# FangjinhuaWang/PatchmatchNet

Hardware: AMD Instinct MI355X
Metric: depth-maps/sec at 1600x1200 N=5 src views (higher is better)
Workload: dtype f32

## Files before the change

### patchmatchnet_amd/csrc/conv_f16s.hip

```cpp
#include "conv_common.hpp"

struct F16sArgs {
    int N, H, W, Ho, Wo, relu;
    int cout, ca;
    float* out_b;
};

template <int CIN, int COUT, int KS, int S, int CC, int CCP, int MT, int WPS, int DIL = 1, int OUTMODE = 0, bool SWAP = (OUTMODE == 0)>
__global__ __launch_bounds__(256, WPS) void conv_f16s_kernel(const float* __restrict__ in, const f16x8* __restrict__ wB,
                                                             const float* __restrict__ shift, float* __restrict__ out,
                                                             const F16sArgs a) {
    constexpr int NT = COUT / 16, NCB = CC / 8, CHUNKS = CIN / CC, NQ = KS * KS * NCB, KSTEPS = (NQ + 3) / 4;
    constexpr int TH = 4 * MT, TW = 16, PH = (TH - 1) * S + (KS - 1) * DIL + 1, PW = (TW - 1) * S + (KS - 1) * DIL + 1;
    constexpr int PAD = DIL * (KS / 2);
    constexpr int PLANE = PH * PW * CCP;
    constexpr int NTHR = 256;
    static_assert(!SWAP || OUTMODE == 0, "swapped operand roles (see the epilogue) serve the channels-last output");
    static_assert(CCP % 8 == 0 && CC % 8 == 0 && CIN % CC == 0, "16-byte aligned channel blocks");
    extern __shared__ float4 f16s_lds4[];
    _Float16* Phi = reinterpret_cast<_Float16*>(f16s_lds4);
    _Float16* Plo = Phi + PLANE;
    const int tid = threadIdx.x, wave = __builtin_amdgcn_readfirstlane(tid >> 6), lane = tid & 63, li = lane & 15, kb = lane >> 4;
    const int tiles_x = (a.Wo + TW - 1) / TW, tiles_y = (a.Ho + TH - 1) / TH;
    const int bt = pmn_xcd_tile(blockIdx.x, a.N * tiles_x * tiles_y);
    const int n = bt / (tiles_x * tiles_y), tr = bt - n * tiles_x * tiles_y;
    const int oy0 = (tr / tiles_x) * TH, ox0 = (tr % tiles_x) * TW;
    const int iy0 = oy0 * S - PAD, ix0 = ox0 * S - PAD;

    f32x4_t accM[MT][NT], accL[MT][NT];
#pragma unroll
    for (int t = 0; t < MT; ++t)
#pragma unroll
        for (int nt = 0; nt < NT; ++nt) {
            accM[t][nt] = f32x4_t{0.f, 0.f, 0.f, 0.f};
            accL[t][nt] = f32x4_t{0.f, 0.f, 0.f, 0.f};
        }

    const f16x8* bl = wB + lane;
    f16x8 bq[2][NT][2];
#pragma unroll
    for (int nt = 0; nt < NT; ++nt) {
        bq[0][nt][0] = bl[(size_t)((0 * NT + nt) * 2 + 0) * 64];
        bq[0][nt][1] = bl[(size_t)((0 * NT + nt) * 2 + 1) * 64];
    }

    const int q4x4 = 4 * (tid % (CC / 4)), pix_first = tid / (CC / 4);
    const int py_first = pix_first / PW, px_first = pix_first - py_first * PW, lds_first = pix_first * CCP + q4x4;

#pragma unroll 1
    for (int ch = 0; ch < CHUNKS; ++ch) {
        if (ch) __syncthreads();
        {
            constexpr int QP = CC / 4, TOT = PH * PW * QP, NL = (TOT + NTHR - 1) / NTHR, SB = 6;
            constexpr int DPIX = NTHR / QP, DY = DPIX / PW, DX = DPIX - DY * PW;
            static_assert(NTHR % QP == 0, "a step of NTHR units is a whole number of pixels");
            const float* src = in + (size_t)n * a.H * a.W * CIN + ch * CC;
            int py = py_first, px = px_first;
#pragma unroll
            for (int k0 = 0; k0 < NL; k0 += SB) {
                float4 v[SB];
#pragma unroll
                for (int k = 0; k < SB; ++k) {
                    const int gy = iy0 + py, gx = ix0 + px;
                    v[k] = make_float4(0.f, 0.f, 0.f, 0.f);
                    if (k0 + k < NL && tid < TOT - (k0 + k) * NTHR && (unsigned)gy < (unsigned)a.H && (unsigned)gx < (unsigned)a.W)
                        v[k] = *reinterpret_cast<const float4*>(src + ((unsigned)(gy * a.W + gx) * CIN + q4x4));
                    px += DX;
                    py += DY;
                    if (px >= PW) {
                        px -= PW;
                        ++py;
                    }
                }
#pragma unroll
                for (int k = 0; k < SB; ++k) {
                    if (k0 + k < NL && tid < TOT - (k0 + k) * NTHR) {
                        f16x4 hi, lo;
                        f16s_split4(v[k], hi, lo);
                        *reinterpret_cast<f16x4*>(Phi + lds_first + (k0 + k) * DPIX * CCP) = hi;
                        *reinterpret_cast<f16x4*>(Plo + lds_first + (k0 + k) * DPIX * CCP) = lo;
                    }
                }
            }
        }
        __syncthreads();

#pragma unroll
        for (int ks = 0; ks < KSTEPS; ++ks) {
            const int cur = ks & 1, nxt = cur ^ 1;
            {
                const int step = ch * KSTEPS + ks + 1;
                const int lim = CHUNKS * KSTEPS - 1;
                const int sidx = step < lim ? step : lim;
#pragma unroll
                for (int nt = 0; nt < NT; ++nt) {
                    bq[nxt][nt][0] = bl[(size_t)((sidx * NT + nt) * 2 + 0) * 64];
                    bq[nxt][nt][1] = bl[(size_t)((sidx * NT + nt) * 2 + 1) * 64];
                }
            }
            int q = 4 * ks + kb;
            if (4 * ks + 3 >= NQ) q = q < NQ - 1 ? q : NQ - 1;
            const int tap = q / NCB, cb = q - tap * NCB;
            const int dy = tap / KS, dx = tap - dy * KS;
            const _Float16* pa = Phi + ((wave * MT * S + dy * DIL) * PW + li * S + dx * DIL) * CCP + cb * 8;
            f16x8 ah[MT], al[MT];
#pragma unroll
            for (int t = 0; t < MT; ++t) {
                ah[t] = *reinterpret_cast<const f16x8*>(pa + t * S * PW * CCP);
                al[t] = *reinterpret_cast<const f16x8*>(pa + t * S * PW * CCP + PLANE);
            }
#pragma unroll
            for (int t = 0; t < MT; ++t)
#pragma unroll
                for (int nt = 0; nt < NT; ++nt)
                    accM[t][nt] = SWAP ? __builtin_amdgcn_mfma_f32_16x16x32_f16(bq[cur][nt][0], ah[t], accM[t][nt], 0, 0, 0)
                                       : __builtin_amdgcn_mfma_f32_16x16x32_f16(ah[t], bq[cur][nt][0], accM[t][nt], 0, 0, 0);
#pragma unroll
            for (int t = 0; t < MT; ++t)
#pragma unroll
                for (int nt = 0; nt < NT; ++nt)
                    accL[t][nt] = SWAP ? __builtin_amdgcn_mfma_f32_16x16x32_f16(bq[cur][nt][1], ah[t], accL[t][nt], 0, 0, 0)
                                       : __builtin_amdgcn_mfma_f32_16x16x32_f16(ah[t], bq[cur][nt][1], accL[t][nt], 0, 0, 0);
#pragma unroll
            for (int t = 0; t < MT; ++t)
#pragma unroll
                for (int nt = 0; nt < NT; ++nt)
                    accL[t][nt] = SWAP ? __builtin_amdgcn_mfma_f32_16x16x32_f16(bq[cur][nt][0], al[t], accL[t][nt], 0, 0, 0)
                                       : __builtin_amdgcn_mfma_f32_16x16x32_f16(al[t], bq[cur][nt][0], accL[t][nt], 0, 0, 0);
            __builtin_amdgcn_sched_barrier(0);
        }
        if (KSTEPS & 1) {
#pragma unroll
            for (int nt = 0; nt < NT; ++nt) {
                bq[0][nt][0] = bq[1][nt][0];
                bq[0][nt][1] = bq[1][nt][1];
            }
        }
    }

    if constexpr (SWAP) {
        const int ox = ox0 + li, oyw = oy0 + wave * MT;
        if (ox < a.Wo) {
            float* po = out + (((size_t)n * a.Ho + oyw) * a.Wo + ox) * COUT + 4 * kb;
            const size_t rs = (size_t)a.Wo * COUT;
            f32x4_t sh[NT];
#pragma unroll
            for (int nt = 0; nt < NT; ++nt) sh[nt] = *reinterpret_cast<const f32x4_t*>(shift + 16 * nt + 4 * kb);
#pragma unroll
            for (int t = 0; t < MT; ++t) {
                if (oyw + t < a.Ho) {
#pragma unroll
                    for (int nt = 0; nt < NT; ++nt) {
                        f32x4_t v = f16s_epilogue(accM[t][nt], accL[t][nt], sh[nt]);
                        if (a.relu) v = f16s_relu(v);
                        *reinterpret_cast<f32x4_t*>(po + t * rs + 16 * nt) = v;
                    }
                }
            }
        }
        return;
    }
#pragma unroll
    for (int nt = 0; nt < NT; ++nt) {
        const int c = nt * 16 + li;
        const float sh = shift[c];
#pragma unroll
        for (int t = 0; t < MT; ++t) {
            const int oy = oy0 + wave * MT + t;
            float v[4];
#pragma unroll
            for (int r = 0; r < 4; ++r) {
                v[r] = f16s_epilogue(accM[t][nt][r], accL[t][nt][r], sh);
                if (a.relu) v[r] = fmaxf(v[r], 0.0f);
            }
            if constexpr (OUTMODE == 0) {
#pragma unroll
                for (int r = 0; r < 4; ++r) {
                    const int ox = ox0 + 4 * kb + r;
                    if (oy < a.Ho && ox < a.Wo) out[(((size_t)n * a.Ho + oy) * a.Wo + ox) * COUT + c] = v[r];
                }
            } else {
                if (c < a.cout && oy < a.Ho) {
                    const bool first = c < a.ca;
                    float* dst = first ? out : a.out_b;
                    const int cx = first ? c : c - a.ca, nc = first ? a.ca : a.cout - a.ca;
                    if constexpr (OUTMODE == 1) {
                        float* row = dst + (((size_t)n * nc + cx) * a.Ho + oy) * a.Wo;
                        const int ox = ox0 + 4 * kb;
                        if ((a.Wo & 3) == 0 && ox + 3 < a.Wo) {
                            *reinterpret_cast<float4*>(row + ox) = make_float4(v[0], v[1], v[2], v[3]);
                        } else {
#pragma unroll
                            for (int r = 0; r < 4; ++r)
                                if (ox + r < a.Wo) row[ox + r] = v[r];
                        }
                    } else {
#pragma unroll
                        for (int r = 0; r < 4; ++r) {
                            const int ox = ox0 + 4 * kb + r;
                            if (ox < a.Wo) dst[(((size_t)n * a.Ho + oy) * a.Wo + ox) * nc + cx] = v[r];
                        }
                    }
                }
            }
        }
    }
}

template <int CIN, int COUT, int KS, int S, int CC, int CCP, int MT, int WPS, int DIL = 1, int OUTMODE = 0, bool SWAP = (OUTMODE == 0)>
static int launch_f16s(const float* in, const void* w, const float* shift, float* out, F16sArgs a, hipStream_t st) {
    constexpr int TH = 4 * MT, PH = (TH - 1) * S + (KS - 1) * DIL + 1, PW = 15 * S + (KS - 1) * DIL + 1;
    const size_t lds = (size_t)2 * PH * PW * CCP * sizeof(_Float16);
    auto kern = conv_f16s_kernel<CIN, COUT, KS, S, CC, CCP, MT, WPS, DIL, OUTMODE, SWAP>;
    if ((size_t)a.H * a.W * CIN >= ((size_t)1 << 30)) return PMN_ERR_SHAPE;
    if (lds > 48 * 1024 && pmn_raise_dynamic_lds(reinterpret_cast<const void*>(kern), lds) != PMN_OK) return PMN_ERR_LAUNCH;
    const int blocks = a.N * ((a.Wo + 15) / 16) * ((a.Ho + TH - 1) / TH);
    PMN_LAUNCH(kern, dim3(blocks), dim3(256), lds, st, in, reinterpret_cast<const f16x8*>(w), shift, out, a);
    PMN_CHECK_LAUNCH();
    return PMN_OK;
}

extern "C" int pmn_conv2d_f16s(const float* in, const void* weights, const float* shift, float* out, int N, int H, int W, int cin,
                               int cout, int k, int stride, int relu, void* stream) {
    if (!in || !weights || !shift || !out || N < 1 || H < 1 || W < 1) return PMN_ERR_ARG;
    F16sArgs a;
    a.N = N; a.H = H; a.W = W; a.relu = relu;
    a.cout = cout; a.ca = cout; a.out_b = nullptr;
    a.Ho = (H - 1) / (stride > 0 ? stride : 1) + 1;
    a.Wo = (W - 1) / (stride > 0 ? stride : 1) + 1;
    hipStream_t st = (hipStream_t)stream;
    if (k == 3 && stride == 1 && cin == 16 && cout == 16) return launch_f16s<16, 16, 3, 1, 16, 16, 4, 4>(in, weights, shift, out, a, st);
    if (k == 3 && stride == 1 && cin == 32 && cout == 32) return launch_f16s<32, 32, 3, 1, 16, 16, 2, 4, 1, 0, false>(in, weights, shift, out, a, st);
    if (k == 3 && stride == 1 && cin == 64 && cout == 64) return launch_f16s<64, 64, 3, 1, 16, 16, 2, 3>(in, weights, shift, out, a, st);
    if (k == 5 && stride == 2 && cin == 8 && cout == 16) return launch_f16s<8, 16, 5, 2, 8, 8, 2, 4>(in, weights, shift, out, a, st);
    if (k == 5 && stride == 2 && cin == 16 && cout == 32) return launch_f16s<16, 32, 5, 2, 8, 8, 2, 4, 1, 0, false>(in, weights, shift, out, a, st);
    if (k == 5 && stride == 2 && cin == 32 && cout == 64) return launch_f16s<32, 64, 5, 2, 16, 24, 2, 2>(in, weights, shift, out, a, st);
    return PMN_ERR_SHAPE;
}


template <int WPS>
__global__ __launch_bounds__(256, WPS) void conv_f16s_pair16_kernel(const float* __restrict__ in, const f16x8* __restrict__ wA,
                                                                   const float* __restrict__ shiftA, const f16x8* __restrict__ wBq,
                                                                   const float* __restrict__ shiftB, float* __restrict__ out,
                                                                   const F16sArgs a) {
    constexpr int C = 16, CCP = 16, NCB = 2, NQ = 18, KSTEPS = 5, TO = 14, RA = 16, PI = 18;
    constexpr int PLANE = PI * PI * CCP;
    extern __shared__ float4 f16s_pair_lds4[];
    _Float16* Phi = reinterpret_cast<_Float16*>(f16s_pair_lds4);
    _Float16* Plo = Phi + PLANE;
    const int tid = threadIdx.x, wave = __builtin_amdgcn_readfirstlane(tid >> 6), lane = tid & 63, li = lane & 15, kb = lane >> 4;
    const int tiles_x = (a.W + TO - 1) / TO, tiles_y = (a.H + TO - 1) / TO;
    const int bt = pmn_xcd_tile(blockIdx.x, a.N * tiles_x * tiles_y);
    const int n = bt / (tiles_x * tiles_y), tr = bt - n * tiles_x * tiles_y;
    const int oy0 = (tr / tiles_x) * TO, ox0 = (tr % tiles_x) * TO;

    {
        constexpr int QP = C / 4, TOT = PI * PI * QP, NL = (TOT + 255) / 256;
        const float* src = in + (size_t)n * a.H * a.W * C;
        float4 v[NL];
#pragma unroll
        for (int k = 0; k < NL; ++k) {
            const int idx = tid + k * 256, pix = idx / QP, q = idx - pix * QP;
            const int py = pix / PI, px = pix - py * PI, gy = oy0 - 2 + py, gx = ox0 - 2 + px;
            v[k] = make_float4(0.f, 0.f, 0.f, 0.f);
            if (idx < TOT && (unsigned)gy < (unsigned)a.H && (unsigned)gx < (unsigned)a.W)
                v[k] = *reinterpret_cast<const float4*>(src + ((unsigned)(gy * a.W + gx) * C + 4 * q));
        }
#pragma unroll
        for (int k = 0; k < NL; ++k) {
            const int idx = tid + k * 256, pix = idx / QP, q = idx - pix * QP;
            if (idx < TOT) {
                f16x4 hi, lo;
                f16s_split4(v[k], hi, lo);
                *reinterpret_cast<f16x4*>(Phi + pix * CCP + 4 * q) = hi;
                *reinterpret_cast<f16x4*>(Plo + pix * CCP + 4 * q) = lo;
            }
        }
    }
    __syncthreads();

    f32x4_t accM[4], accL[4];
    auto layer = [&](const f16x8* __restrict__ wq, const int pitch) {
        const f16x8* bl = wq + lane;
        f16x8 bq[2][2];
        bq[0][0] = bl[0];
        bq[0][1] = bl[64];
#pragma unroll
        for (int t = 0; t < 4; ++t) {
            accM[t] = f32x4_t{0.f, 0.f, 0.f, 0.f};
            accL[t] = f32x4_t{0.f, 0.f, 0.f, 0.f};
        }
#pragma unroll
        for (int ks = 0; ks < KSTEPS; ++ks) {
            const int cur = ks & 1, nxt = cur ^ 1;
            const int sidx = ks + 1 < KSTEPS ? ks + 1 : KSTEPS - 1;
            bq[nxt][0] = bl[(size_t)(sidx * 2 + 0) * 64];
            bq[nxt][1] = bl[(size_t)(sidx * 2 + 1) * 64];
            int q = 4 * ks + kb;
            if (4 * ks + 3 >= NQ) q = q < NQ - 1 ? q : NQ - 1;
            const int tap = q / NCB, cb = q - tap * NCB;
            const int dy = tap / 3, dx = tap - dy * 3;
            const _Float16* pa = Phi + ((wave * 4 + dy) * pitch + li + dx) * CCP + cb * 8;
            f16x8 ah[4], al[4];
#pragma unroll
            for (int t = 0; t < 4; ++t) {
                ah[t] = *reinterpret_cast<const f16x8*>(pa + t * pitch * CCP);
                al[t] = *reinterpret_cast<const f16x8*>(pa + t * pitch * CCP + PLANE);
            }
#pragma unroll
            for (int t = 0; t < 4; ++t) accM[t] = __builtin_amdgcn_mfma_f32_16x16x32_f16(bq[cur][0], ah[t], accM[t], 0, 0, 0);
#pragma unroll
            for (int t = 0; t < 4; ++t) accL[t] = __builtin_amdgcn_mfma_f32_16x16x32_f16(bq[cur][1], ah[t], accL[t], 0, 0, 0);
#pragma unroll
            for (int t = 0; t < 4; ++t) accL[t] = __builtin_amdgcn_mfma_f32_16x16x32_f16(bq[cur][0], al[t], accL[t], 0, 0, 0);
            __builtin_amdgcn_sched_barrier(0);
        }
    };

    layer(wA, PI);
    f16x4 rh[4], rl[4];
    {
        const f32x4_t sh = *reinterpret_cast<const f32x4_t*>(shiftA + 4 * kb);
        const int gx = ox0 - 1 + li;
#pragma unroll
        for (int t = 0; t < 4; ++t) {
            const int gy = oy0 - 1 + wave * 4 + t;
            f32x4_t v = f16s_epilogue(accM[t], accL[t], sh);
            if (a.relu) v = f16s_relu(v);
            if (!((unsigned)gy < (unsigned)a.H && (unsigned)gx < (unsigned)a.W)) v = f32x4_t{0.f, 0.f, 0.f, 0.f};
            f16s_split4(v, rh[t], rl[t]);
        }
    }
    __syncthreads();
#pragma unroll
    for (int t = 0; t < 4; ++t) {
        const int pix = (wave * 4 + t) * RA + li;
        *reinterpret_cast<f16x4*>(Phi + pix * CCP + 4 * kb) = rh[t];
        *reinterpret_cast<f16x4*>(Plo + pix * CCP + 4 * kb) = rl[t];
    }
    __syncthreads();

    layer(wBq, RA);
    {
        const int ox = ox0 + li;
        if (li < TO && ox < a.W) {
            const f32x4_t sh = *reinterpret_cast<const f32x4_t*>(shiftB + 4 * kb);
#pragma unroll
            for (int t = 0; t < 4; ++t) {
                const int r = wave * 4 + t, oy = oy0 + r;
                if (r < TO && oy < a.H) {
                    f32x4_t v = f16s_epilogue(accM[t], accL[t], sh);
                    if (a.relu) v = f16s_relu(v);
                    *reinterpret_cast<f32x4_t*>(out + (((size_t)n * a.H + oy) * a.W + ox) * C + 4 * kb) = v;
                }
            }
        }
    }
}

extern "C" int pmn_conv2d_f16s_pair(const float* in, const void* weights_a, const float* shift_a, const void* weights_b,
                                    const float* shift_b, float* out, int N, int H, int W, int channels, int relu, void* stream) {
    if (!in || !weights_a || !shift_a || !weights_b || !shift_b || !out || N < 1 || H < 1 || W < 1) return PMN_ERR_ARG;
    if (channels != 16) return PMN_ERR_SHAPE;
    if ((size_t)H * W * 16 >= ((size_t)1 << 30)) return PMN_ERR_SHAPE;
    F16sArgs a;
    a.N = N; a.H = H; a.W = W; a.Ho = H; a.Wo = W; a.relu = relu;
    a.cout = 16; a.ca = 16; a.out_b = nullptr;
    const size_t lds = (size_t)2 * 18 * 18 * 16 * sizeof(_Float16);
    const int blocks = N * ((W + 13) / 14) * ((H + 13) / 14);
    PMN_LAUNCH(conv_f16s_pair16_kernel<4>, dim3(blocks), dim3(256), lds, (hipStream_t)stream, in, reinterpret_cast<const f16x8*>(weights_a),
               shift_a, reinterpret_cast<const f16x8*>(weights_b), shift_b, out, a);
    PMN_CHECK_LAUNCH();
    return PMN_OK;
}


template <int CIN, int DIL, int MT, int WPS>
static int dispatch_heads(const float* in, const void* w, const float* shift, float* out_a, int coutp, F16sArgs a, hipStream_t st) {
    if (coutp == 32) return launch_f16s<CIN, 32, 3, 1, 16, 16, MT, WPS, DIL, 1>(in, w, shift, out_a, a, st);
    if (coutp == 48) return launch_f16s<CIN, 48, 3, 1, 16, 16, MT, WPS, DIL, 1>(in, w, shift, out_a, a, st);
    if (coutp == 64) return launch_f16s<CIN, 64, 3, 1, 16, 16, MT, (WPS > 3 ? 3 : WPS), DIL, 1>(in, w, shift, out_a, a, st);
    return PMN_ERR_SHAPE;
}

extern "C" int pmn_offset_heads_f16s(const float* in, const void* weights, const float* shift, float* out_a, float* out_b, int N, int H,
                                     int W, int cin, int cout, int ca, int dil, void* stream) {
    if (!in || !weights || !shift || !out_a || N < 1 || H < 1 || W < 1 || cout < 1 || ca < 1 || ca > cout) return PMN_ERR_ARG;
    if (ca < cout && !out_b) return PMN_ERR_ARG;
    F16sArgs a;
    a.N = N; a.H = H; a.W = W; a.Ho = H; a.Wo = W; a.relu = 0;
    a.cout = cout; a.ca = ca; a.out_b = out_b;
    const int coutp = (cout + 15) / 16 * 16;
    hipStream_t st = (hipStream_t)stream;
    if (cin == 64 && dil == 2) return dispatch_heads<64, 2, 2, 3>(in, weights, shift, out_a, coutp, a, st);
    if (cin == 32 && dil == 4) return dispatch_heads<32, 4, 2, 4>(in, weights, shift, out_a, coutp, a, st);
    if (cin == 16 && dil == 6) return dispatch_heads<16, 6, 2, 4>(in, weights, shift, out_a, coutp, a, st);
    return PMN_ERR_SHAPE;
}

#ifndef PMN_STEM_TH
#define PMN_STEM_TH 32
#endif
template <bool VEC4, int TH>
__global__ __launch_bounds__(256, 4) void stem_f16s_kernel(const float* __restrict__ img, const float* __restrict__ w0,
                                                          const float* __restrict__ s0, const f16x8* __restrict__ w1A,
                                                          const float* __restrict__ s1, float* __restrict__ out, const int N,
                                                          const int H, const int W, const float* const* __restrict__ img_tab,
                                                          const int BV) {
    constexpr int TS = 16, IW = TH + 4, XS = 24, MW = TS + 2, MRP = 18, MROWS = TH + 2, NTHR = 256;
    static_assert(TH % 16 == 0, "a wave owns TH / 4 rows, four at a time");
    __shared__ float4 xin4[3 * IW * (XS / 4)];
    __shared__ float4 mid4[2 * MROWS * MRP];
    float* xin = reinterpret_cast<float*>(xin4);
    _Float16* midh = reinterpret_cast<_Float16*>(mid4);
    _Float16* midl = midh + MROWS * MRP * 8;
    typedef const float __attribute__((address_space(4))) cfloat;
    const cfloat* cw0 = (const cfloat*)w0;
    const cfloat* cs0 = (const cfloat*)s0;
    const int tid = threadIdx.x, wave = __builtin_amdgcn_readfirstlane(tid >> 6), lane = tid & 63, li = lane & 15, kb = lane >> 4;
    const int tiles_x = (W + TS - 1) / TS, tiles_y = (H + TH - 1) / TH;
    const int bt = pmn_xcd_tile(blockIdx.x, N * tiles_x * tiles_y);
    const int n = bt / (tiles_x * tiles_y), tr = bt - n * tiles_x * tiles_y;
    const int oy0 = (tr / tiles_x) * TH, ox0 = (tr % tiles_x) * TS;
    if (img_tab) img = img_tab[n / BV] + (ptrdiff_t)((n % BV) - n) * 3 * H * W;

    f16x8 wa[3][2];
#pragma unroll
    for (int ks = 0; ks < 3; ++ks) {
        wa[ks][0] = w1A[(ks * 2 + 0) * 64 + lane];
        wa[ks][1] = w1A[(ks * 2 + 1) * 64 + lane];
    }
    if constexpr (VEC4) {
        constexpr int NU = (3 * IW + 31) / 32;
        float4 v[NU];
        const int j = tid & 7, gx = ox0 - 4 + 4 * j;
#pragma unroll
        for (int u = 0; u < NU; ++u) {
            const int R = (tid >> 3) + 32 * u;
            const int c = (R >= IW) + (R >= 2 * IW), r = R - IW * c, gy = oy0 - 2 + r;
            v[u] = make_float4(0.f, 0.f, 0.f, 0.f);
            if (j < 6 && R < 3 * IW && (unsigned)gy < (unsigned)H && (unsigned)gx < (unsigned)W)
                v[u] = *reinterpret_cast<const float4*>(img + (((size_t)n * 3 + c) * H + gy) * W + gx);
        }
#pragma unroll
        for (int u = 0; u < NU; ++u) {
            const int R = (tid >> 3) + 32 * u;
            if (j < 6 && R < 3 * IW) xin4[R * (XS / 4) + j] = v[u];
        }
    } else {
        constexpr int NU = (3 * IW + 7) / 8;
        float v[NU];
        const int q = tid & 31, gx = ox0 - 4 + q;
#pragma unroll
        for (int u = 0; u < NU; ++u) {
            const int R = (tid >> 5) + 8 * u;
            const int c = (R >= IW) + (R >= 2 * IW), r = R - IW * c, gy = oy0 - 2 + r;
            v[u] = 0.0f;
            if (q < XS && R < 3 * IW && (unsigned)gy < (unsigned)H && (unsigned)gx < (unsigned)W)
                v[u] = img[(((size_t)n * 3 + c) * H + gy) * W + gx];
        }
#pragma unroll
        for (int u = 0; u < NU; ++u) {
            const int R = (tid >> 5) + 8 * u;
            if (q < XS && R < 3 * IW) xin[R * XS + q] = v[u];
        }
    }
    __syncthreads();
    for (int m = tid; m < MW * MROWS; m += NTHR) {
        const int r = m / MW, q = m - r * MW;
        const int gy = oy0 - 1 + r, gx = ox0 - 1 + q;
        f16x8 hi = {0, 0, 0, 0, 0, 0, 0, 0}, lo = {0, 0, 0, 0, 0, 0, 0, 0};
        if ((unsigned)gy < (unsigned)H && (unsigned)gx < (unsigned)W) {
            float acc[8];
#pragma unroll
            for (int c = 0; c < 8; ++c) acc[c] = 0.0f;
            const float* xp = xin + r * XS + q + 2;
#pragma unroll 1
            for (int ky = 0; ky < 3; ++ky) {
                const cfloat* wq = cw0 + __builtin_amdgcn_readfirstlane(ky * 72);
#pragma unroll
                for (int kx = 0; kx < 3; ++kx)
#pragma unroll
                    for (int ci = 0; ci < 3; ++ci) {
                        const float v = xp[(ci * IW + ky) * XS + kx];
#pragma unroll
                        for (int c = 0; c < 8; ++c) acc[c] = fmaf(v, wq[(kx * 3 + ci) * 8 + c], acc[c]);
                    }
            }
#pragma unroll
            for (int c = 0; c < 8; c += 2) {
                const f32x2_t x = {fmaxf(acc[c] + cs0[c], 0.0f), fmaxf(acc[c + 1] + cs0[c + 1], 0.0f)};
                const f16x2_t h = f16s_hi2(x), l = f16s_lo2(x, h);
                hi[c] = h[0];
                hi[c + 1] = h[1];
                lo[c] = l[0];
                lo[c + 1] = l[1];
            }
        }
        *reinterpret_cast<f16x8*>(midh + (r * MRP + q) * 8) = hi;
        *reinterpret_cast<f16x8*>(midl + (r * MRP + q) * 8) = lo;
    }
    __syncthreads();
#pragma unroll 1
    for (int rg = 0; rg < TH / 16; ++rg) {
    const int wrow = wave * (TH / 4) + 4 * rg;
    f32x4_t accM[4], accL[4];
#pragma unroll
    for (int t = 0; t < 4; ++t) {
        accM[t] = f32x4_t{0.f, 0.f, 0.f, 0.f};
        accL[t] = f32x4_t{0.f, 0.f, 0.f, 0.f};
    }
#pragma unroll
    for (int ks = 0; ks < 3; ++ks) {
        int q = 4 * ks + kb;
        q = q < 8 ? q : 8;
        const int dy = q / 3, dx = q - dy * 3;
        const _Float16* pb = midh + ((wrow + dy) * MRP + li + dx) * 8;
        f16x8 bh[4], blo[4];
#pragma unroll
        for (int t = 0; t < 4; ++t) {
            bh[t] = *reinterpret_cast<const f16x8*>(pb + t * MRP * 8);
            blo[t] = *reinterpret_cast<const f16x8*>(pb + t * MRP * 8 + MROWS * MRP * 8);
        }
#pragma unroll
        for (int t = 0; t < 4; ++t) accM[t] = __builtin_amdgcn_mfma_f32_16x16x32_f16(wa[ks][0], bh[t], accM[t], 0, 0, 0);
#pragma unroll
        for (int t = 0; t < 4; ++t) accL[t] = __builtin_amdgcn_mfma_f32_16x16x32_f16(wa[ks][0], blo[t], accL[t], 0, 0, 0);
#pragma unroll
        for (int t = 0; t < 4; ++t) accL[t] = __builtin_amdgcn_mfma_f32_16x16x32_f16(wa[ks][1], bh[t], accL[t], 0, 0, 0);
    }
    const int ox = ox0 + li, oyw = oy0 + wrow;
    if (kb < 2 && ox < W) {
        const f32x4_t sh = *reinterpret_cast<const f32x4_t*>(s1 + 4 * kb);
        float* po = out + (((size_t)n * H + oyw) * W + ox) * 8 + 4 * kb;
        const size_t rs = (size_t)W * 8;
#pragma unroll
        for (int t = 0; t < 4; ++t) {
            if (oyw + t < H) {
                *reinterpret_cast<f32x4_t*>(po + t * rs) = f16s_relu(f16s_epilogue(accM[t], accL[t], sh));
            }
        }
    }
    }
}

static int launch_stem_f16s(const float* img, const float* const* img_table, int B, bool vec4, const float* w0, const float* s0,
                            const void* w1a, const float* s1, float* out, int N, int H, int W, void* stream) {
    constexpr int TS = 16, TH = PMN_STEM_TH;
    const int blocks = N * ((W + TS - 1) / TS) * ((H + TH - 1) / TH);
    PMN_LAUNCH((vec4 ? stem_f16s_kernel<true, PMN_STEM_TH> : stem_f16s_kernel<false, PMN_STEM_TH>), dim3(blocks), dim3(256), 0,
               (hipStream_t)stream, img, w0, s0, reinterpret_cast<const f16x8*>(w1a), s1, out, N, H, W, img_table, B);
    PMN_CHECK_LAUNCH();
    return PMN_OK;
}

extern "C" int pmn_stem_f16s(const float* img, const float* w0, const float* s0, const void* w1a, const float* s1, float* out,
                             int N, int H, int W, void* stream) {
    if (!img || !w0 || !s0 || !w1a || !s1 || !out || N < 1 || H < 1 || W < 1) return PMN_ERR_ARG;
    const bool vec4 = W % 4 == 0 && (reinterpret_cast<uintptr_t>(img) & 15) == 0;
    return launch_stem_f16s(img, nullptr, 1, vec4, w0, s0, w1a, s1, out, N, H, W, stream);
}

extern "C" int pmn_stem_f16s_views(const float* const* img_table, int views, const float* w0, const float* s0, const void* w1a,
                                   const float* s1, float* out, int B, int H, int W, void* stream) {
    if (!img_table || !w0 || !s0 || !w1a || !s1 || !out || views < 1 || B < 1 || H < 1 || W < 1) return PMN_ERR_ARG;
    return launch_stem_f16s(nullptr, img_table, B, W % 4 == 0, w0, s0, w1a, s1, out, views * B, H, W, stream);
}
```

Baseline: 396.5.

## Pipeline next input-chunk patch loads under MFMAs in f16s conv kernel

```diff
diff --git a/patchmatchnet_amd/csrc/conv_f16s.hip b/patchmatchnet_amd/csrc/conv_f16s.hip
--- a/patchmatchnet_amd/csrc/conv_f16s.hip
+++ b/patchmatchnet_amd/csrc/conv_f16s.hip
@@ -4,21 +4,34 @@
     int N, H, W, Ho, Wo, relu;
     int cout, ca;
     float* out_b;
+    int pipe = 0;
 };
 
-template <int CIN, int COUT, int KS, int S, int CC, int CCP, int MT, int WPS, int DIL = 1, int OUTMODE = 0, bool SWAP = (OUTMODE == 0)>
-__global__ __launch_bounds__(256, WPS) void conv_f16s_kernel(const float* __restrict__ in, const f16x8* __restrict__ wB,
-                                                             const float* __restrict__ shift, float* __restrict__ out,
-                                                             const F16sArgs a) {
+__host__ __device__ constexpr bool f16s_two_buffers(int plane_halves, int wps) {
+    return (size_t)2 * (2 * plane_halves * sizeof(_Float16)) * wps <= (size_t)160 * 1024;
+}
+#ifndef PMN_F16S_PIPE_ALL
+#define PMN_F16S_PIPE_ALL 0
+#endif
+__host__ __device__ constexpr bool f16s_pipe_shape(int cin, int cout, int ks, int cc, int dil) {
+    if (cin / cc < 2) return false;
+    if (PMN_F16S_PIPE_ALL) return true;
+    return ks == 5 && cin == 32 && cout == 64;
+}
+
+template <int CIN, int COUT, int KS, int S, int CC, int CCP, int MT, int WPS, int DIL, int OUTMODE, bool SWAP, bool PIPE>
+__device__ __forceinline__ void conv_f16s_body(const float* __restrict__ in, const f16x8* __restrict__ wB,
+                                               const float* __restrict__ shift, float* __restrict__ out, const F16sArgs& a,
+                                               _Float16* const Phi) {
     constexpr int NT = COUT / 16, NCB = CC / 8, CHUNKS = CIN / CC, NQ = KS * KS * NCB, KSTEPS = (NQ + 3) / 4;
     constexpr int TH = 4 * MT, TW = 16, PH = (TH - 1) * S + (KS - 1) * DIL + 1, PW = (TW - 1) * S + (KS - 1) * DIL + 1;
     constexpr int PAD = DIL * (KS / 2);
     constexpr int PLANE = PH * PW * CCP;
     constexpr int NTHR = 256;
+    constexpr bool TWO = PIPE && f16s_two_buffers(PLANE, WPS);
     static_assert(!SWAP || OUTMODE == 0, "swapped operand roles (see the epilogue) serve the channels-last output");
     static_assert(CCP % 8 == 0 && CC % 8 == 0 && CIN % CC == 0, "16-byte aligned channel blocks");
-    extern __shared__ float4 f16s_lds4[];
-    _Float16* Phi = reinterpret_cast<_Float16*>(f16s_lds4);
+    static_assert(!PIPE || CHUNKS > 1, "the pipelined form prefetches the next chunk");
     _Float16* Plo = Phi + PLANE;
     const int tid = threadIdx.x, wave = __builtin_amdgcn_readfirstlane(tid >> 6), lane = tid & 63, li = lane & 15, kb = lane >> 4;
     const int tiles_x = (a.Wo + TW - 1) / TW, tiles_y = (a.Ho + TH - 1) / TH;
@@ -47,44 +60,68 @@
     const int q4x4 = 4 * (tid % (CC / 4)), pix_first = tid / (CC / 4);
     const int py_first = pix_first / PW, px_first = pix_first - py_first * PW, lds_first = pix_first * CCP + q4x4;
 
-#pragma unroll 1
-    for (int ch = 0; ch < CHUNKS; ++ch) {
-        if (ch) __syncthreads();
-        {
-            constexpr int QP = CC / 4, TOT = PH * PW * QP, NL = (TOT + NTHR - 1) / NTHR, SB = 6;
-            constexpr int DPIX = NTHR / QP, DY = DPIX / PW, DX = DPIX - DY * PW;
-            static_assert(NTHR % QP == 0, "a step of NTHR units is a whole number of pixels");
-            const float* src = in + (size_t)n * a.H * a.W * CIN + ch * CC;
+    constexpr int QP = CC / 4, TOT = PH * PW * QP, NL = (TOT + NTHR - 1) / NTHR, SB = PIPE ? NL : 6;
+    constexpr int DPIX = NTHR / QP, DY = DPIX / PW, DX = DPIX - DY * PW;
+    static_assert(NTHR % QP == 0, "a step of NTHR units is a whole number of pixels");
+    auto patch_load = [&](const int ch, const int k0, float4(&v)[SB], int& py, int& px) __attribute__((always_inline)) {
+        const float* src = in + (size_t)n * a.H * a.W * CIN + ch * CC;
+#pragma unroll
+        for (int k = 0; k < SB; ++k) {
+            const int gy = iy0 + py, gx = ix0 + px;
+            if constexpr (PIPE) {
+                const int cy = min(max(gy, 0), a.H - 1), cx = min(max(gx, 0), a.W - 1);
+                v[k] = *reinterpret_cast<const float4*>(src + ((unsigned)(cy * a.W + cx) * CIN + q4x4));
+            } else {
+                v[k] = make_float4(0.f, 0.f, 0.f, 0.f);
+                if (k0 + k < NL && tid < TOT - (k0 + k) * NTHR && (unsigned)gy < (unsigned)a.H && (unsigned)gx < (unsigned)a.W)
+                    v[k] = *reinterpret_cast<const float4*>(src + ((unsigned)(gy * a.W + gx) * CIN + q4x4));
+            }
+            px += DX;
+            py += DY;
+            if (px >= PW) {
+                px -= PW;
+                ++py;
+            }
+        }
+    };
+    auto patch_store = [&](const int k0, float4(&v)[SB], const int boff) __attribute__((always_inline)) {
+        if constexpr (PIPE) {
             int py = py_first, px = px_first;
 #pragma unroll
-            for (int k0 = 0; k0 < NL; k0 += SB) {
-                float4 v[SB];
-#pragma unroll
-                for (int k = 0; k < SB; ++k) {
-                    const int gy = iy0 + py, gx = ix0 + px;
-                    v[k] = make_float4(0.f, 0.f, 0.f, 0.f);
-                    if (k0 + k < NL && tid < TOT - (k0 + k) * NTHR && (unsigned)gy < (unsigned)a.H && (unsigned)gx < (unsigned)a.W)
-                        v[k] = *reinterpret_cast<const float4*>(src + ((unsigned)(gy * a.W + gx) * CIN + q4x4));
-                    px += DX;
-                    py += DY;
-                    if (px >= PW) {
-                        px -= PW;
-                        ++py;
-                    }
+            for (int k = 0; k < SB; ++k) {
+                if (!((unsigned)(iy0 + py) < (unsigned)a.H && (unsigned)(ix0 + px) < (unsigned)a.W)) v[k] = make_float4(0.f, 0.f, 0.f, 0.f);
+                px += DX;
+                py += DY;
+                if (px >= PW) {
+                    px -= PW;
+                    ++py;
                 }
-#pragma unroll
-                for (int k = 0; k < SB; ++k) {
-                    if (k0 + k < NL && tid < TOT - (k0 + k) * NTHR) {
-                        f16x4 hi, lo;
-                        f16s_split4(v[k], hi, lo);
-                        *reinterpret_cast<f16x4*>(Phi + lds_first + (k0 + k) * DPIX * CCP) = hi;
-                        *reinterpret_cast<f16x4*>(Plo + lds_first + (k0 + k) * DPIX * CCP) = lo;
-                    }
-                }
-            }
-        }
-        __syncthreads();
-
+            }
+            static_assert(TOT > NTHR, "every thread has a first unit");
+#pragma unroll
+            for (int k = 0; k < SB; ++k) {
+                const bool last = k > 0 && TOT - k * NTHR < NTHR, own = !last || tid < TOT - k * NTHR;
+                const float4 x = own ? v[k] : v[k > 0 ? k - 1 : 0];
+                const int slot = boff + lds_first + (own ? k : k - 1) * DPIX * CCP;
+                f16x4 hi, lo;
+                f16s_split4(x, hi, lo);
+                *reinterpret_cast<f16x4*>(Phi + slot) = hi;
+                *reinterpret_cast<f16x4*>(Plo + slot) = lo;
+            }
+            return;
+        }
+#pragma unroll
+        for (int k = 0; k < SB; ++k) {
+            if (k0 + k < NL && tid < TOT - (k0 + k) * NTHR) {
+                f16x4 hi, lo;
+                f16s_split4(v[k], hi, lo);
+                *reinterpret_cast<f16x4*>(Phi + boff + lds_first + (k0 + k) * DPIX * CCP) = hi;
+                *reinterpret_cast<f16x4*>(Plo + boff + lds_first + (k0 + k) * DPIX * CCP) = lo;
+            }
+        }
+    };
+
+    auto k_loop = [&](const int ch, const int boff, auto&& under_mfmas) __attribute__((always_inline)) {
 #pragma unroll
         for (int ks = 0; ks < KSTEPS; ++ks) {
             const int cur = ks & 1, nxt = cur ^ 1;
@@ -98,11 +135,16 @@
                     bq[nxt][nt][1] = bl[(size_t)((sidx * NT + nt) * 2 + 1) * 64];
                 }
             }
+            if (PIPE && ks == 0) {
+                __builtin_amdgcn_sched_barrier(0);
+                under_mfmas();
+                __builtin_amdgcn_sched_barrier(0);
+            }
             int q = 4 * ks + kb;
             if (4 * ks + 3 >= NQ) q = q < NQ - 1 ? q : NQ - 1;
             const int tap = q / NCB, cb = q - tap * NCB;
             const int dy = tap / KS, dx = tap - dy * KS;
-            const _Float16* pa = Phi + ((wave * MT * S + dy * DIL) * PW + li * S + dx * DIL) * CCP + cb * 8;
+            const _Float16* pa = Phi + boff + ((wave * MT * S + dy * DIL) * PW + li * S + dx * DIL) * CCP + cb * 8;
             f16x8 ah[MT], al[MT];
 #pragma unroll
             for (int t = 0; t < MT; ++t) {
@@ -136,6 +178,40 @@
                 bq[0][nt][1] = bq[1][nt][1];
             }
         }
+    };
+
+    if constexpr (!PIPE) {
+#pragma unroll 1
+        for (int ch = 0; ch < CHUNKS; ++ch) {
+            if (ch) __syncthreads();
+            int py = py_first, px = px_first;
+#pragma unroll
+            for (int k0 = 0; k0 < NL; k0 += SB) {
+                float4 v[SB];
+                patch_load(ch, k0, v, py, px);
+                patch_store(k0, v, 0);
+            }
+            __syncthreads();
+            k_loop(ch, 0, [] {});
+        }
+    } else {
+        float4 v[NL];
+        int py = py_first, px = px_first;
+        patch_load(0, 0, v, py, px);
+        patch_store(0, v, 0);
+#pragma unroll 1
+        for (int ch = 0; ch < CHUNKS - 1; ++ch) {
+            const int boff = TWO ? (ch & 1) * 2 * PLANE : 0;
+            __syncthreads();
+            k_loop(ch, boff, [&]() __attribute__((always_inline)) {
+                py = py_first, px = px_first;
+                patch_load(ch + 1, 0, v, py, px);
+            });
+            if (!TWO) __syncthreads();
+            patch_store(0, v, TWO ? 2 * PLANE - boff : 0);
+        }
+        __syncthreads();
+        k_loop(CHUNKS - 1, TWO ? ((CHUNKS - 1) & 1) * 2 * PLANE : 0, [] {});
     }
 
     if constexpr (SWAP) {
@@ -208,9 +284,30 @@
 }
 
 template <int CIN, int COUT, int KS, int S, int CC, int CCP, int MT, int WPS, int DIL = 1, int OUTMODE = 0, bool SWAP = (OUTMODE == 0)>
+__global__ __launch_bounds__(256, WPS) void conv_f16s_kernel(const float* __restrict__ in, const f16x8* __restrict__ wB,
+                                                             const float* __restrict__ shift, float* __restrict__ out,
+                                                             const F16sArgs a) {
+    extern __shared__ float4 f16s_lds4[];
+    _Float16* const lds = reinterpret_cast<_Float16*>(f16s_lds4);
+    if constexpr (f16s_pipe_shape(CIN, COUT, KS, CC, DIL)) {
+        if (a.pipe) {
+            conv_f16s_body<CIN, COUT, KS, S, CC, CCP, MT, WPS, DIL, OUTMODE, SWAP, true>(in, wB, shift, out, a, lds);
+            return;
+        }
+    }
+    conv_f16s_body<CIN, COUT, KS, S, CC, CCP, MT, WPS, DIL, OUTMODE, SWAP, false>(in, wB, shift, out, a, lds);
+}
+
+static bool f16s_pipeline_enabled() {
+    const char* e = getenv("PMN_F16S_PIPELINE");
+    return !(e && e[0] == '0' && e[1] == '\0');
+}
+
+template <int CIN, int COUT, int KS, int S, int CC, int CCP, int MT, int WPS, int DIL = 1, int OUTMODE = 0, bool SWAP = (OUTMODE == 0)>
 static int launch_f16s(const float* in, const void* w, const float* shift, float* out, F16sArgs a, hipStream_t st) {
     constexpr int TH = 4 * MT, PH = (TH - 1) * S + (KS - 1) * DIL + 1, PW = 15 * S + (KS - 1) * DIL + 1;
-    const size_t lds = (size_t)2 * PH * PW * CCP * sizeof(_Float16);
+    a.pipe = f16s_pipe_shape(CIN, COUT, KS, CC, DIL) && f16s_pipeline_enabled();
+    const size_t lds = (size_t)2 * PH * PW * CCP * sizeof(_Float16) * (a.pipe && f16s_two_buffers(PH * PW * CCP, WPS) ? 2 : 1);
     auto kern = conv_f16s_kernel<CIN, COUT, KS, S, CC, CCP, MT, WPS, DIL, OUTMODE, SWAP>;
     if ((size_t)a.H * a.W * CIN >= ((size_t)1 << 30)) return PMN_ERR_SHAPE;
     if (lds > 48 * 1024 && pmn_raise_dynamic_lds(reinterpret_cast<const void*>(kern), lds) != PMN_OK) return PMN_ERR_LAUNCH;
```

Result: no change. 394.3 (-0.6%).
